# LorienLV/genarchbench

Measured on AMD Instinct MI355X. Metric: bsw ROI M alignments/sec, higher is better.
Workload: dtype i16/i32; 1 GPU; bsw-large; total_items=10000000

## Files before the change

genarchbench_amd/csrc/bsw.hip:

```cpp
#include "gab_internal.h"
#include <atomic>
#include <algorithm>
#include <new>
#include <string.h>
#include <time.h>
#include <stdlib.h>

namespace {

constexpr int kQBuckets = 256;
constexpr int kTBuckets = 256;
constexpr int kNumKeys = kQBuckets * kTBuckets;
constexpr int kClassStep = 16;
constexpr int kNumClasses = kQBuckets / kClassStep;
constexpr int kSlices = 2;
constexpr int64_t kSlice0 = 1 << 20;
constexpr int64_t kSliceMin = 1 << 22;
constexpr int kSortGridBeside = 256;
static_assert(kSliceMin >= (1 << 21) && kSlice0 < kSliceMin && kSlice0 >= 64 * 8192, "slice 0 has to fill the chip with its class launches, and calls below 2^21 pairs stay unsliced");

struct BswConst {
    int32_t o_del, e_del, o_ins, e_ins, zdrop, end_bonus, w, max_sc;
    uint32_t row_lo[5];
    uint32_t row_hi[5];
};

struct BswStats {
    unsigned long long cells;
    int32_t max_h0[kNumClasses];
    int32_t bad;
    int32_t first_bad;
};
GAB_STATIC_ATOMIC64(BswStats, cells);

struct BswIO {
    const uint8_t *ref; const int64_t *ref_off;
    const uint8_t *qry; const int64_t *qry_off;
    const int32_t *len1, *len2, *h0;
    int64_t ref_bytes, qry_bytes, n;
    int64_t ref_lo, qry_lo;
    int64_t ref_hi, qry_hi;
};

__device__ __forceinline__ int bsw_key(int qlen, int tlen, int h0) {
    int tb = tlen >> 3; if (tb > kTBuckets / 4 - 1) tb = kTBuckets / 4 - 1;
    int hc = h0 >> 5; if (hc > 3) hc = 3;
    return (qlen - 1) * kTBuckets + tb * 4 + hc;
}

__device__ __forceinline__ int bsw_hslot(int key) { return (int)(((uint32_t)key * 4099u) & (uint32_t)(kNumKeys - 1)); }
static_assert((kNumKeys & (kNumKeys - 1)) == 0, "bsw_hslot needs a power-of-two key space");

__global__ __launch_bounds__(256) void bsw_hist(BswIO io, int64_t lo, int64_t hi, uint32_t *hist, uint32_t *rank, BswStats *st) {
    __shared__ int cls_h0[kNumClasses];
    if (threadIdx.x < kNumClasses) cls_h0[threadIdx.x] = 0;
    __syncthreads();
    int64_t i = lo + (int64_t)blockIdx.x * blockDim.x + threadIdx.x;
    int64_t stride = (int64_t)gridDim.x * blockDim.x;
    for (; i < hi; i += stride) {
        int ql = io.len2[i], tl = io.len1[i], h = io.h0[i];
        int64_t ro = io.ref_off[i], qo = io.qry_off[i];
        bool ok = ql >= 1 && ql <= GAB_BSW_MAX_QLEN && tl >= 1 && tl <= GAB_BSW_MAX_TLEN && h >= 0 &&
                  h <= (1 << 29) && ro >= io.ref_lo && qo >= io.qry_lo &&
                  ro + tl + 3 <= io.ref_bytes && qo + ql + 3 <= io.qry_bytes &&
                  ro + tl <= io.ref_hi && qo + ql <= io.qry_hi;
        if (!ok) {
            atomicAdd(&st->bad, 1);
            atomicMin((unsigned int *)&st->first_bad, (unsigned int)(i + 1 > 0x7fffffff ? 0x7fffffff : i + 1));
            rank[i] = ~0u;
            continue;
        }
        if (h > 0) atomicMax(&cls_h0[(ql - 1) / kClassStep], h);
        rank[i] = atomicAdd(&hist[bsw_hslot(bsw_key(ql, tl, h))], 1u);
    }
    __syncthreads();
    if (threadIdx.x < kNumClasses && cls_h0[threadIdx.x] > 0) atomicMax(&st->max_h0[threadIdx.x], cls_h0[threadIdx.x]);
}

constexpr int kScanBlocks = kNumKeys / 1024;
static_assert(kScanBlocks == 64, "bsw_scan_b reduces the block totals with one wave");
__global__ __launch_bounds__(1024) void bsw_scan_a(const uint32_t *__restrict__ hist, uint32_t *__restrict__ start, uint32_t *__restrict__ sums) {
    __shared__ uint32_t wsum[16];
    const int t = threadIdx.x, key = blockIdx.x * 1024 + t, lane = t & 63, wv = t >> 6;
    const uint32_t v = hist[bsw_hslot(key)];
    uint32_t inc = v;
    for (int o = 1; o < 64; o <<= 1) { const uint32_t u = __shfl_up(inc, o); if (lane >= o) inc += u; }
    if (lane == 63) wsum[wv] = inc;
    __syncthreads();
    uint32_t before = 0;
    for (int k = 0; k < wv; k++) before += wsum[k];
    start[key] = before + inc - v;
    if (t == 1023) sums[blockIdx.x] = before + inc;
}
__global__ __launch_bounds__(1024) void bsw_scan_b(uint32_t *__restrict__ start, const uint32_t *__restrict__ sums, uint32_t *__restrict__ qstart) {
    __shared__ uint32_t s_off, s_total;
    const int t = threadIdx.x, key = blockIdx.x * 1024 + t;
    if (t < 64) {
        const uint32_t sv = sums[t];
        uint32_t mine = t < (int)blockIdx.x ? sv : 0, all = sv;
        for (int o = 32; o > 0; o >>= 1) { mine += __shfl_xor(mine, o); all += __shfl_xor(all, o); }
        if (t == 0) { s_off = mine; s_total = all; }
    }
    __syncthreads();
    const uint32_t run = start[key] + s_off;
    start[key] = run;
    if ((key % kTBuckets) == 0) qstart[key / kTBuckets] = run;
    if (key == kNumKeys - 1) { start[kNumKeys] = s_total; qstart[kQBuckets] = s_total; }
}

struct __attribute__((aligned(32))) BswRec { int64_t ref_off, qry_off; int32_t len1, len2, h0; uint32_t id; };

__global__ __launch_bounds__(256) void bsw_scatter(BswIO io, int64_t lo, int64_t hi, const uint32_t *__restrict__ start,
                                                   const uint32_t *__restrict__ rank, BswRec *recs) {
    int64_t i = lo + (int64_t)blockIdx.x * blockDim.x + threadIdx.x;
    int64_t stride = (int64_t)gridDim.x * blockDim.x;
    for (; i < hi; i += stride) {
        int ql = io.len2[i], tl = io.len1[i];
        if (rank[i] == ~0u) continue;
        BswRec r;
        r.ref_off = io.ref_off[i]; r.qry_off = io.qry_off[i]; r.len1 = tl; r.len2 = ql; r.h0 = io.h0[i]; r.id = (uint32_t)i;
        recs[start[bsw_key(ql, tl, r.h0)] + rank[i]] = r;
    }
}

__device__ __forceinline__ uint32_t load_u32_unaligned(const uint8_t *p) {
    uint32_t w;
    __builtin_memcpy(&w, p, 4);
    return w;
}

template <bool WIDE>
__global__ __launch_bounds__(64) void bsw_dp(BswIO io, BswConst c, const BswRec *__restrict__ recs,
                                            int64_t kbeg, int64_t kend, int qcap,
                                            int32_t *__restrict__ score_out,
                                            gab_bsw_result *__restrict__ result_out, BswStats *st) {
    extern __shared__ uint32_t lds[];
    const int lane = threadIdx.x;
    const int64_t k = kbeg + (int64_t)(gridDim.x - 1 - blockIdx.x) * 64 + lane;
    const bool valid = k < kend;
    BswRec rec; rec.ref_off = rec.qry_off = 0; rec.len1 = rec.len2 = rec.h0 = 0; rec.id = 0u;
    if (valid) rec = recs[k];
    const uint32_t id = rec.id;

    uint32_t *const H = lds + lane;
    uint32_t *const E = lds + (size_t)(qcap + 1) * 64 + lane;
    uint8_t *const QC = reinterpret_cast<uint8_t *>(lds + (size_t)(WIDE ? 2 : 1) * (qcap + 1) * 64) + lane * 4;

    unsigned long long cells = 0;
    if (valid) {
        const int qlen = rec.len2, tlen = rec.len1, h0 = rec.h0;
        const uint8_t *q = io.qry + rec.qry_off;
        const uint8_t *t = io.ref + rec.ref_off;
        const int oe_del = c.o_del + c.e_del, oe_ins = c.o_ins + c.e_ins;
        const int e_del = c.e_del, e_ins = c.e_ins;

        for (int w4 = 0; w4 * 4 < qlen; w4++)
            *reinterpret_cast<uint32_t *>(QC + w4 * 256) = load_u32_unaligned(q + w4 * 4);

        int w = c.w;
        {
            int lim = (int)((double)(qlen * c.max_sc + c.end_bonus - c.o_ins) / e_ins + 1.);
            lim = lim > 1 ? lim : 1; w = w < lim ? w : lim;
            lim = (int)((double)(qlen * c.max_sc + c.end_bonus - c.o_del) / e_del + 1.);
            lim = lim > 1 ? lim : 1; w = w < lim ? w : lim;
        }
        const bool score_only = result_out == nullptr;
        bool prune = score_only && (qlen <= w + 1 || h0 - oe_ins - (w + 1) * e_ins <= 0) && (c.zdrop == 0 || c.zdrop >= 8 * c.max_sc);
        int best, best_i, best_j, g_i, gscore, max_off;
      for (;;) {
        {
            int prev = h0;
            for (int j = 0; j <= qlen; j++) {
                int v;
                if (j == 0) v = h0;
                else if (j == 1) v = h0 > oe_ins ? h0 - oe_ins : 0;
                else v = prev > e_ins ? prev - e_ins : 0;
                prev = v;
                H[j * 64] = (uint32_t)v;
                if (WIDE) E[j * 64] = 0u;
            }
        }
        best = h0; best_i = -1; best_j = -1; g_i = -1; gscore = -1; max_off = 0;
        int beg = 0, end = qlen;
        int stale_pot = 0;
        bool dropped = false, abandon = false;
        uint32_t tw = load_u32_unaligned(t);
        for (int i = 0; i < tlen; i++) {
            const int tc = (tw >> ((i & 3) * 8)) & 0xff;
            if ((i & 3) == 3 && i + 1 < tlen) tw = load_u32_unaligned(t + i + 1);
            uint32_t rlo = c.row_lo[4], rhi = c.row_hi[4];
            rlo = tc == 0 ? c.row_lo[0] : rlo; rhi = tc == 0 ? c.row_hi[0] : rhi;
            rlo = tc == 1 ? c.row_lo[1] : rlo; rhi = tc == 1 ? c.row_hi[1] : rhi;
            rlo = tc == 2 ? c.row_lo[2] : rlo; rhi = tc == 2 ? c.row_hi[2] : rhi;
            rlo = tc == 3 ? c.row_lo[3] : rlo; rhi = tc == 3 ? c.row_hi[3] : rhi;

            if (beg < i - w) beg = i - w;
            if (end > i + w + 1) { end = i + w + 1; stale_pot = max(stale_pot, best + c.max_sc * (qlen - end)); }
            if (end > qlen) end = qlen;
            const int beg0 = beg, end0 = end;
            int hleft = 0;
            if (beg == 0) { hleft = h0 - (c.o_del + e_del * (i + 1)); hleft = hleft > 0 ? hleft : 0; }
            int f = 0;
            uint32_t rowpk = 0;
            int rowmax32 = 0, rowmax_j = -1;
            int j = beg;
            for (; j < end; j++) {
                int diag, e;
                if (WIDE) { diag = (int)H[j * 64]; e = (int)E[j * 64]; }
                else { uint32_t v = H[j * 64]; diag = (int)(v & 0xffffu); e = (int)(v >> 16); }
                uint32_t qc = QC[(j >> 2) * 256 + (j & 3)];
                qc = qc > 4u ? 4u : qc;
                int sc = (int)__builtin_amdgcn_perm(rhi, rlo, qc | 0x0c0c0c00u) - 128;
                int M = diag ? diag + sc : 0;
                int h = max(max(M, e), f);
                int t1 = M - oe_del; t1 = t1 > 0 ? t1 : 0;
                int en = e - e_del; en = en > t1 ? en : t1;
                if (WIDE) { H[j * 64] = (uint32_t)hleft; E[j * 64] = (uint32_t)en; }
                else H[j * 64] = (uint32_t)hleft | ((uint32_t)en << 16);
                hleft = h;
                if (WIDE) {
                    if (!(rowmax32 > h)) rowmax_j = j;
                    rowmax32 = h > rowmax32 ? h : rowmax32;
                } else {
                    uint32_t pk = ((uint32_t)h << 16) | (uint32_t)j;
                    rowpk = pk > rowpk ? pk : rowpk;
                }
                int t2 = M - oe_ins; t2 = t2 > 0 ? t2 : 0;
                f -= e_ins; f = f > t2 ? f : t2;
            }
            cells += (unsigned)(end > beg ? end - beg : 0);
            int rowmax;
            if (WIDE) rowmax = rowmax32;
            else { rowmax = (int)(rowpk >> 16); rowmax_j = end > beg ? (int)(rowpk & 0xffffu) : -1; }
            if (WIDE) { H[end * 64] = (uint32_t)hleft; E[end * 64] = 0u; }
            else H[end * 64] = (uint32_t)hleft;
            if (j == qlen) {
                if (!(gscore > hleft)) g_i = i;
                gscore = hleft > gscore ? hleft : gscore;
            }
            if (rowmax == 0) {
                if (dropped && beg == 0) {
                    const int hb = h0 - c.o_del - e_del * (i + 1);
                    abandon = hb > 0 && hb + c.max_sc * min(tlen - 1 - i, qlen) > best;
                }
                break;
            }
            const int rows_left = tlen - 1 - i;
            bool try_exit = false;
            if (rowmax > best) {
                best = rowmax; best_i = i; best_j = rowmax_j;
                int off = rowmax_j - i; off = off < 0 ? -off : off;
                max_off = off > max_off ? off : max_off;
            } else {
                if (c.zdrop > 0) {
                    if (dropped && rowmax < best - c.zdrop) { abandon = true; break; }
                    int di = i - best_i, dj = rowmax_j - best_j;
                    if (di > dj) { if (best - rowmax - (di - dj) * e_del > c.zdrop) break; }
                    else { if (best - rowmax - (dj - di) * e_ins > c.zdrop) break; }
                }
                try_exit = score_only && rowmax + c.max_sc * min(rows_left, qlen - 1 - rowmax_j) <= best;
            }
            if (dropped && end < qlen && end != i + w + 1 && hleft > e_ins &&
                hleft - e_ins + c.max_sc * min(rows_left, qlen - end - 1) > best) { abandon = true; break; }
            if (WIDE) {
                for (j = beg; j < end && H[j * 64] == 0u && E[j * 64] == 0u; j++) {}
                beg = j;
                for (j = end; j >= beg && H[j * 64] == 0u && E[j * 64] == 0u; j--) {}
            } else {
                for (j = beg; j < end && H[j * 64] == 0u; j++) {}
                beg = j;
                for (j = end; j >= beg && H[j * 64] == 0u; j--) {}
            }
            int jl = j;
            end = j + 2 < qlen ? j + 2 : qlen;
            if (prune && beg < end) {
                bool go = true;
                if (beg == 0) {
                    const int hb = h0 - c.o_del - e_del * (i + 2);
                    go = hb <= 0 || hb + c.max_sc * min(rows_left, qlen) <= best;
                }
                if (go) {
                    const int lcap = min(end, beg0 + 4);
                    for (j = beg; j < lcap; j++) {
                        const int m = WIDE ? max((int)H[j * 64], (int)E[j * 64]) : max((int)(H[j * 64] & 0xffffu), (int)(H[j * 64] >> 16));
                        if (m && m + c.max_sc * min(rows_left, qlen - j) > best) break;
                    }
                    dropped = dropped || j > beg;
                    beg = j;
                }
            }
            if (prune && jl >= beg) {
                const int from = jl;
                for (; jl >= beg && jl > end0 - 4; jl--) {
                    const int m = WIDE ? max((int)H[jl * 64], (int)E[jl * 64]) : max((int)(H[jl * 64] & 0xffffu), (int)(H[jl * 64] >> 16));
                    if (m && m + c.max_sc * min(rows_left, qlen - jl) > best) break;
                    H[jl * 64] = 0u;
                    if (WIDE) E[jl * 64] = 0u;
                }
                if (jl < from) { dropped = true; end = jl + 2 < qlen ? jl + 2 : qlen; }
            }
            if (try_exit) {
                int bound = stale_pot;
                if (beg == 0) {
                    const int hb = h0 - c.o_del - e_del * (i + 2);
                    if (hb > 0) bound = max(bound, hb + c.max_sc * min(rows_left, qlen));
                }
                for (j = beg; j <= end && bound <= best; j++) {
                    const int hd = WIDE ? (int)H[j * 64] : (int)(H[j * 64] & 0xffffu);
                    if (hd) bound = max(bound, hd + c.max_sc * min(rows_left, qlen - j));
                }
                if (bound <= best) break;
            }
        }
        if (!abandon) break;
        prune = false;
      }
        score_out[id] = best;
        if (result_out) {
            gab_bsw_result r;
            r.score = best; r.qle = best_j + 1; r.tle = best_i + 1;
            r.gtle = g_i + 1; r.gscore = gscore; r.max_off = max_off;
            result_out[id] = r;
        }
    }
    for (int o = 32; o > 0; o >>= 1) cells += __shfl_xor(cells, o);
    if (lane == 0 && cells) atomicAdd(&st->cells, cells);
}

// ... 52 lines not shown
    asm("v_sub_u16 %0, %2, %3\n\tv_max_i16_sdwa %0, %1, %0 dst_sel:WORD_0 dst_unused:UNUSED_PAD src0_sel:WORD_1 src1_sel:WORD_0"
        : "=&v"(r) : "v"(t), "v"(f), "v"(e));
    return r;
}
__device__ __forceinline__ uint32_t rowkey_fold(uint32_t key, uint32_t a, uint32_t b, uint32_t c, uint32_t j) {
    uint32_t t;
    asm("v_max_i16 %1, %2, %3\n\tv_max_i16 %1, %1, %4\n\tv_lshl_or_b32 %1, %1, 16, %5\n\tv_max_u32 %0, %0, %1"
        : "+v"(key), "=&v"(t) : "v"(a), "v"(b), "v"(c), "v"(j));
    return key;
}
struct BswCellOut { int h, en, f; };
__device__ __forceinline__ BswCellOut bsw_cell(int diag, int e, int f, uint32_t qc, uint32_t rlo, uint32_t rhi, int oe_del,
                                               int e_del, int oe_ins, int e_ins) {
    const int sc = (int)__builtin_amdgcn_perm(rhi, rlo, qc | 0x0c0c0c00u) - 128;
    const int M = diag ? diag + sc : 0;
    BswCellOut o;
    o.h = max(max(M, e), f);
    o.en = max(max(M - oe_del, e - e_del), 0);
    o.f = max(max(M - oe_ins, f - e_ins), 0);
    return o;
}

template <bool SYM, bool MS1, bool SO>
__global__ __launch_bounds__(64) void bsw_dp8(BswIO io, BswConst c, const BswRec *__restrict__ recs, int64_t kbeg,
                                              int64_t kend, int qcap, int32_t *__restrict__ score_out,
                                              gab_bsw_result *__restrict__ result_out, BswStats *st) {
    extern __shared__ uint32_t lds[];
    __shared__ __attribute__((aligned(8))) uint32_t row_tab[10];
    if (threadIdx.x < 5) { row_tab[2 * threadIdx.x] = c.row_lo[threadIdx.x]; row_tab[2 * threadIdx.x + 1] = c.row_hi[threadIdx.x]; }
    __syncthreads();
    const int lane = threadIdx.x;
    const int64_t k = kbeg + (int64_t)(gridDim.x - 1 - blockIdx.x) * 64 + lane;
    const bool valid = k < kend;
    BswRec rec; rec.ref_off = rec.qry_off = 0; rec.len1 = rec.len2 = rec.h0 = 0; rec.id = 0u;
    if (valid) rec = recs[k];
    const uint32_t id = rec.id;
    const int ncell_dw = (qcap + 2) / 2;
    uint8_t *const CB = reinterpret_cast<uint8_t *>(lds + lane);
    uint32_t *const CW = lds + lane;
    uint8_t *const QN = reinterpret_cast<uint8_t *>(lds + (size_t)ncell_dw * 64) + lane;
#define CELL16(j) (*reinterpret_cast<uint16_t *>(CB + ((j) >> 1) * 256 + ((j) & 1) * 2))
#define QPAIR(p) (QN[(p) * 64])

    unsigned long long cells = 0;
    if (valid) {
        const int qlen = rec.len2, tlen = rec.len1, h0 = rec.h0;
        const uint8_t *q = io.qry + rec.qry_off;
        const uint8_t *t = io.ref + rec.ref_off;
        const int oe_del = c.o_del + c.e_del, oe_ins = c.o_ins + c.e_ins;
        const int e_del = c.e_del, e_ins = c.e_ins;

        for (int p0 = 0; p0 * 2 < qlen; p0 += 4) {
            const uint32_t s0 = load_u32_unaligned(q + p0 * 2);
            const uint32_t s1 = p0 * 2 + 4 < qlen ? load_u32_unaligned(q + p0 * 2 + 4) : 0u;
            const uint32_t n0 = pk_min_u16(s0 & 0x00ff00ffu, 0x00040004u) | pk_min_u16((s0 >> 8) & 0x00ff00ffu, 0x00040004u) << 4;
            const uint32_t n1 = pk_min_u16(s1 & 0x00ff00ffu, 0x00040004u) | pk_min_u16((s1 >> 8) & 0x00ff00ffu, 0x00040004u) << 4;
            QPAIR(p0) = (uint8_t)n0; QPAIR(p0 + 1) = (uint8_t)(n0 >> 16);
            QPAIR(p0 + 2) = (uint8_t)n1; QPAIR(p0 + 3) = (uint8_t)(n1 >> 16);
        }
        int w = c.w;
        {
            int lim = (int)((double)(qlen * c.max_sc + c.end_bonus - c.o_ins) / e_ins + 1.);
            lim = lim > 1 ? lim : 1; w = w < lim ? w : lim;
            lim = (int)((double)(qlen * c.max_sc + c.end_bonus - c.o_del) / e_del + 1.);
            lim = lim > 1 ? lim : 1; w = w < lim ? w : lim;
        }
        uint32_t k_selz = 0x0c000c00u, k_lo8 = 0x00ff00ffu, v_e_ins = (uint32_t)e_ins;
        uint32_t k_cstep = 512u, k_qstep = 128u, k_jstep = 4u;
        asm volatile("" : "+v"(k_selz), "+v"(k_lo8), "+v"(v_e_ins), "+v"(k_cstep), "+v"(k_qstep), "+v"(k_jstep));
        bool prune = SO && (qlen <= w + 1 || h0 - oe_ins - (w + 1) * e_ins <= 0) && (c.zdrop == 0 || c.zdrop >= 8 * c.max_sc);
        int best, best_i, best_j, g_i, gscore, max_off;
      for (;;) {
        {
            int v = h0 - oe_ins;
            CW[0] = (uint32_t)h0 | (uint32_t)max(v, 0) << 16;
            for (int p = 1; p <= (qlen >> 1); p++) {
                const int lo = v - e_ins;
                v = lo - e_ins;
                CW[p * 64] = (uint32_t)max(lo, 0) | (uint32_t)max(v, 0) << 16;
            }
        }
        best = h0; best_i = -1; best_j = -1; g_i = -1; gscore = -1; max_off = 0;
        int beg = 0, end = qlen;
        int hrow = h0 - c.o_del - e_del;
        int stale_pot = 0;
        bool dropped = false, abandon = false;
        uint32_t tw = load_u32_unaligned(t);
        for (int i = 0; i < tlen; i++, hrow -= e_del) {
            const int tc = (tw >> ((i & 3) * 8)) & 0xff;
            if ((i & 3) == 3 && i + 1 < tlen) tw = load_u32_unaligned(t + i + 1);
            const uint2 rr = *reinterpret_cast<const uint2 *>(&row_tab[2 * (tc < 4 ? tc : 4)]);
            const uint32_t rlo = rr.x, rhi = rr.y;
            if (beg < i - w) beg = i - w;
            if (end > i + w + 1) { end = i + w + 1; stale_pot = max(stale_pot, best + mul24(c.max_sc, qlen - end)); }
            if (end > qlen) end = qlen;
            int hleft = 0;
            if (beg == 0) hleft = hrow > 0 ? hrow : 0;
            int f = 0;
            uint32_t rowpk = 0;
            int j = beg;
            uint32_t *cw = CW + (j >> 1) * 64;
            const uint8_t *qp = QN + (j >> 1) * 64;
            uint32_t v0 = cw[0], q0 = qp[0];
            {
                const uint32_t vn = cw[64], qn = qp[64];
                if ((j & 1) && j < end) {
                    const BswCellOut o = bsw_cell((int)((v0 >> 16) & 0xff), (int)(v0 >> 24), f, q0 >> 4, rlo, rhi, oe_del, e_del,
                                                  oe_ins, e_ins);
                    CELL16(j) = (uint16_t)(hleft | o.en << 8);
                    hleft = o.h; f = o.f;
                    rowpk = ((uint32_t)o.h << 16) | (uint32_t)j;
                    j++;
                    v0 = vn; q0 = qn; cw += 64; qp += 64;
                }
            }
            if (j + 1 < end) {
                const uint32_t k_oe_del = as_u32(pk_splat(oe_del)), k_e_del = as_u32(pk_splat(e_del));
                const uint32_t k_oe_ins = as_u32(pk_splat(oe_ins));
                const uint32_t k_bias = 0x00800080u, k_nib = 0x000f000fu;
// ... 36 lines not shown
                }
                if (j + 1 < end) {
                    const uint32_t v1 = cl[64], q1 = ql[64];
                    uint32_t hj;
                    BSW_PAIR(v0, q0, cl[0], hj)
                    const uint32_t pa = (hj << 16) | (uint32_t)j, pb = (HB << 16) | (uint32_t)(j + 1);
                    rowpk = max(max(rowpk, pa), pb);
                    j += 2; v0 = v1; q0 = q1;
                }
                hleft = (int)HB; f = (int)FV;
#undef BSW_PAIR
            }
            if (j < end) {
                const BswCellOut o = bsw_cell((int)(v0 & 0xff), (int)((v0 >> 8) & 0xff), f, q0 & 0xfu, rlo, rhi, oe_del, e_del,
                                              oe_ins, e_ins);
                CELL16(j) = (uint16_t)(hleft | o.en << 8);
                hleft = o.h; f = o.f;
                const uint32_t pk = ((uint32_t)o.h << 16) | (uint32_t)j;
                rowpk = pk > rowpk ? pk : rowpk;
                j++;
            }
            cells += (unsigned)(end > beg ? end - beg : 0);
            const int rowmax = (int)(rowpk >> 16);
            CELL16(end) = (uint16_t)hleft;
            if constexpr (!SO) {
                if (j == qlen) {
                    if (!(gscore > hleft)) g_i = i;
                    gscore = hleft > gscore ? hleft : gscore;
                }
            }
            if (rowmax == 0) {
                if constexpr (SO) {
                    if (dropped && beg == 0) {
                        abandon = hrow > 0 && hrow + mul24(c.max_sc, min(tlen - 1 - i, qlen)) > best;
                    }
                }
                break;
            }
            const int kj = (int)(rowpk & 0xffffu);
            const int pb = beg >> 1, pe = end >> 1;
            const uint32_t *const rw = CW + ((kj + 1) >> 1) * 64;
            const uint32_t r0 = rw[0], r1 = rw[64], r2 = rw[128];
            const uint32_t b0 = CW[pb * 64], b1 = CW[(pb + 1) * 64], b2 = CW[(pb + 2) * 64];
            const uint32_t e2 = CW[pe * 64], e1 = CW[(pe > 0 ? pe - 1 : 0) * 64], e0 = CW[(pe > 1 ? pe - 2 : 0) * 64];
            int rowmax_j;
            {
                const uint32_t sh = (uint32_t)((kj + 1) & 1) << 4;
                const uint32_t c01 = __builtin_amdgcn_alignbit(r1, r0, sh), c23 = __builtin_amdgcn_alignbit(r2, r1, sh);
                const uint32_t rm2 = (uint32_t)rowmax * 0x00010001u;
                const uint32_t ne = __builtin_amdgcn_perm(pk_min_u16_1((c23 ^ rm2) & 0x00ff00ffu), pk_min_u16_1((c01 ^ rm2) & 0x00ff00ffu),
                                                          0x06040200u);
                const int nv = end - kj < 4 ? end - kj : 4;
                const uint32_t eq = (ne ^ 0x01010101u) & (0x01010101u >> (8 * (4 - nv)));
                rowmax_j = kj + ((31 - __builtin_clz(eq)) >> 3);
            }
            const int rows_left = tlen - 1 - i;
            const bool raised = rowmax > best;
            bool stop = false;
            if (c.zdrop > 0) {
                const int di = i - best_i, dj = rowmax_j - best_j;
                const int gap = di > dj ? mul24(di - dj, e_del) : mul24(dj - di, e_ins);
                stop = !raised && best - rowmax - gap > c.zdrop;
                if constexpr (SO) {
                    abandon = !raised && dropped && rowmax < best - c.zdrop;
                    stop = stop || abandon;
                }
            }
            const bool try_exit = SO && !raised && rowmax + mul24(c.max_sc, min(rows_left, qlen - 1 - rowmax_j)) <= best;
            if (raised) {
                best = rowmax; best_i = i; best_j = rowmax_j;
                if constexpr (!SO) {
                    int off = rowmax_j - i; off = off < 0 ? -off : off;
                    max_off = off > max_off ? off : max_off;
                }
            }
            if constexpr (SO) {
                const bool guard = !stop && dropped && end < qlen && end != i + w + 1 && hleft > e_ins &&
                                   hleft - e_ins + mul24(c.max_sc, min(rows_left, qlen - end - 1)) > best;
                abandon = abandon || guard;
                stop = stop || guard;
            }
            int edge_pot = 0;
            {
                const int beg0 = beg, end0 = end;
                uint64_t x = (uint64_t)b1 << 32 | b0;
                if (beg0 & 1) x = (x >> 16) | (uint64_t)(b2 & 0xffffu) << 48;
                uint64_t y = (uint64_t)e2 << 32 | e1;
                if (!(end0 & 1)) y = (y << 16) | (e0 >> 16);
                const int lz = x ? __builtin_ctzll(x) >> 4 : 4, tz = y ? __builtin_clzll(y) >> 4 : 4;
                int base = min(beg0 + lz, end0);
                int lp = lz, tp = tz;
                if constexpr (SO) {
                    const int rq = min(rows_left, qlen);
                    const int hb = hrow - e_del;
                    edge_pot = hb > 0 ? hb + mul24(c.max_sc, rq) : 0;
                    const bool go = prune && base < qlen && (base != 0 || edge_pot <= best);
                    const uint32_t r2 = as_u32(pk_splat(rq)), m2 = as_u32(pk_splat(c.max_sc));
                    const uint32_t bestL = (uint32_t)(go ? best : 0) * 0x00010001u, bestR = (uint32_t)(prune ? best : 0) * 0x00010001u;
                    const uint32_t cl01 = ((uint32_t)(qlen - beg0) & 0xffffu) | (uint32_t)(qlen - beg0 - 1) << 16;
                    const uint32_t cr01 = ((uint32_t)(qlen - end0 + 3) & 0xffffu) | (uint32_t)(qlen - end0 + 2) << 16;
#define BSW_STAY(W, CL, B2, OUT)                                                                                   \
    {                                                                                                             \
        const uint32_t m = pk_max_i16((W) & 0x00ff00ffu, ((W) >> 8) & 0x00ff00ffu);                              \
        (OUT) = pk_mul_lo(pk_subsat_u16_v(add_u32_v(m, pk_mul_lo(pk_min_u16((CL), r2), m2)), (B2)), pk_min_u16_1(m)); \
    }
                    uint32_t sll, slh, srl, srh;
                    BSW_STAY((uint32_t)x, cl01, bestL, sll)
                    BSW_STAY((uint32_t)(x >> 32), cl01 - 0x00020002u, bestL, slh)
                    BSW_STAY((uint32_t)y, cr01, bestR, srl)
                    BSW_STAY((uint32_t)(y >> 32), cr01 - 0x00020002u, bestR, srh)
#undef BSW_STAY
                    const uint64_t stl = (uint64_t)slh << 32 | sll, str = (uint64_t)srh << 32 | srl;
                    lp = stl ? __builtin_ctzll(stl) >> 4 : 4;
                    tp = str ? __builtin_clzll(str) >> 4 : 4;
                }
                int bl = beg0 + lp;
                if (__builtin_expect(lz == 4, 0)) {
                    for (j = beg0 + 4; j < end0 && CELL16(j) == 0; j++) {}
                    base = bl = j < end0 ? j : end0;
                }
                j = end0 - tz;
                if (__builtin_expect(tz == 4, 0)) for (; j >= base && CELL16(j) == 0; j--) {}
                const int jlz = j > base - 1 ? j : base - 1;
                const int endz = jlz + 2 < qlen ? jlz + 2 : qlen;
                beg = bl < endz ? bl : endz;
                int jl = jlz;
                if constexpr (SO) {
                    dropped = dropped || beg > base;
                    int jn = end0 - tp;
                    jn = jn > beg - 1 ? jn : beg - 1;
                    dropped = dropped || jn < jlz;
// ... 77 lines not shown
    hipStream_t aux[kAux] = {nullptr};
    hipEvent_t fork = nullptr, join[kAux] = {nullptr};
    hipStream_t sort = nullptr;
    hipEvent_t sort_fork = nullptr, sort_join = nullptr;
    bool have_stats = false;
    int stat_slices = 1;
    uint32_t *h_qstart[kSlices] = {nullptr};
    BswStats *h_stats[kSlices] = {nullptr};
    BswStats *h_init = nullptr;
    bool out_of_order = false;
};

extern "C" int gab_bsw_create(const gab_bsw_params *p, int device, gab_bsw **out) {
    if (!p || !out) { gab_set_error("gab_bsw_create: NULL argument"); return GAB_EINVAL; }
    *out = nullptr;
    GAB_CHECK(p->e_del > 0 && p->e_ins > 0 && p->o_del >= 0 && p->o_ins >= 0,
              "gab_bsw_create: gap penalties must be o>=0, e>0 (got o_del=%d e_del=%d o_ins=%d e_ins=%d)",
              p->o_del, p->e_del, p->o_ins, p->e_ins);
    GAB_CHECK(p->w >= 0 && p->zdrop >= 0, "gab_bsw_create: w and zdrop must be >= 0");
    GAB_CHECK(p->o_del + p->e_del < 32768 && p->o_ins + p->e_ins < 32768 && p->end_bonus >= -32768 &&
              p->end_bonus < 32768, "gab_bsw_create: penalties out of 16-bit range");
    int rc = gab_check_device(device);
    if (rc) return rc;
    gab_device_guard g(device);
    gab_bsw *h = new (std::nothrow) gab_bsw();
    if (!h) { gab_set_error("out of host memory"); return GAB_ENOMEM; }
    h->device = device; h->prm = *p;
    BswConst &c = h->cst;
    c.o_del = p->o_del; c.e_del = p->e_del; c.o_ins = p->o_ins; c.e_ins = p->e_ins;
    c.zdrop = p->zdrop; c.end_bonus = p->end_bonus; c.w = p->w;
    int mx = 0;
    for (int k = 0; k < 25; k++) mx = p->mat[k] > mx ? p->mat[k] : mx;
    c.max_sc = mx;
    for (int t = 0; t < 5; t++) {
        uint32_t lo = 0;
        for (int q = 0; q < 4; q++) lo |= (uint32_t)(uint8_t)(p->mat[t * 5 + q] + 128) << (8 * q);
        c.row_lo[t] = lo;
        c.row_hi[t] = (uint32_t)(uint8_t)(p->mat[t * 5 + 4] + 128);
    }
    for (int k = 0; k < 4; k++)
        if (hipEventCreate(&h->ev[k]) != hipSuccess) { gab_set_error("hipEventCreate failed"); delete h; return GAB_EDEVICE; }
    bool aux_ok = hipEventCreateWithFlags(&h->fork, hipEventDisableTiming) == hipSuccess;
    for (int k = 0; k < gab_bsw::kAux && aux_ok; k++)
        aux_ok = hipStreamCreateWithFlags(&h->aux[k], hipStreamNonBlocking) == hipSuccess &&
                 hipEventCreateWithFlags(&h->join[k], hipEventDisableTiming) == hipSuccess;
    if (!aux_ok) { gab_set_error("gab_bsw_create: stream / event creation failed"); delete h; return GAB_EDEVICE; }
    if (hipFuncSetAttribute((const void *)bsw_dp<false>, hipFuncAttributeMaxDynamicSharedMemorySize, 160 * 1024) != hipSuccess ||
        hipFuncSetAttribute((const void *)bsw_dp<true>, hipFuncAttributeMaxDynamicSharedMemorySize, 160 * 1024) != hipSuccess) {
        gab_set_error("hipFuncSetAttribute(MaxDynamicSharedMemorySize) failed"); delete h; return GAB_EDEVICE;
    }
    for (int k = 0; k < 8; k++)
        if (hipFuncSetAttribute((const void *)bsw_dp8_kernel(k & 4, k & 2, k & 1), hipFuncAttributeMaxDynamicSharedMemorySize, 160 * 1024 - 64) != hipSuccess) {
            gab_set_error("hipFuncSetAttribute(MaxDynamicSharedMemorySize) failed"); delete h; return GAB_EDEVICE;
        }
    if (hipHostMalloc((void **)&h->h_qstart[0], sizeof(uint32_t) * (kQBuckets + 1) * kSlices) != hipSuccess ||
        hipHostMalloc((void **)&h->h_stats[0], sizeof(BswStats) * (kSlices + 1)) != hipSuccess) {
        gab_set_error("hipHostMalloc failed"); gab_bsw_destroy(h); return GAB_ENOMEM;
    }
    for (int k = 1; k < kSlices; k++) { h->h_qstart[k] = h->h_qstart[0] + (size_t)k * (kQBuckets + 1); h->h_stats[k] = h->h_stats[0] + k; }
    h->h_init = h->h_stats[0] + kSlices;
    memset(h->h_init, 0, sizeof(BswStats));
    h->h_init->first_bad = 0x7fffffff;
    *out = h;
    return GAB_OK;
}

extern "C" void gab_bsw_destroy(gab_bsw *h) {
    if (!h) return;
    gab_device_guard g(h->device);
    h->ws.release(); h->io.release(); h->hs.release();
    for (int k = 0; k < 4; k++) if (h->ev[k]) (void)hipEventDestroy(h->ev[k]);
    if (h->fork) (void)hipEventDestroy(h->fork);
    for (int k = 0; k < gab_bsw::kAux; k++) {
        if (h->join[k]) (void)hipEventDestroy(h->join[k]);
        if (h->aux[k]) (void)hipStreamDestroy(h->aux[k]);
    }
    if (h->sort_fork) (void)hipEventDestroy(h->sort_fork);
    if (h->sort_join) (void)hipEventDestroy(h->sort_join);
    if (h->sort) (void)hipStreamDestroy(h->sort);
    if (h->h_qstart[0]) (void)hipHostFree(h->h_qstart[0]);
    if (h->h_stats[0]) (void)hipHostFree(h->h_stats[0]);
    delete h;
}

struct BswLayout {
    size_t o_start, o_qstart, o_sums, o_stats, blk;
    size_t o_recs, o_rank, total;
    explicit BswLayout(size_t n) {
        o_start = sizeof(uint32_t) * kNumKeys;
        o_qstart = o_start + sizeof(uint32_t) * (kNumKeys + 1);
        o_sums = o_qstart + sizeof(uint32_t) * (kQBuckets + 1);
        o_stats = (o_sums + sizeof(uint32_t) * kScanBlocks + 15) & ~(size_t)15;
        blk = (o_stats + sizeof(BswStats) + 255) & ~(size_t)255;
        o_recs = blk * kSlices;
        o_rank = o_recs + ((sizeof(BswRec) * n + 255) & ~(size_t)255);
        total = o_rank + sizeof(uint32_t) * n;
    }
};

static int bsw_run_device_impl(gab_bsw *h, const uint8_t *ref, int64_t ref_bytes, const int64_t *ref_off,
                               const uint8_t *qry, int64_t qry_bytes, const int64_t *qry_off,
                               const int32_t *len1, const int32_t *len2, const int32_t *h0, int64_t n,
                               int32_t *score_out, gab_bsw_result *result_out, void *stream_, int64_t ref_lo, int64_t qry_lo,
                               int64_t ref_hi, int64_t qry_hi);
extern "C" int gab_bsw_run_device(gab_bsw *h, const uint8_t *ref, int64_t ref_bytes, const int64_t *ref_off,
                                  const uint8_t *qry, int64_t qry_bytes, const int64_t *qry_off,
                                  const int32_t *len1, const int32_t *len2, const int32_t *h0, int64_t n,
                                  int32_t *score_out, gab_bsw_result *result_out, void *stream_) {
    if (h) gab_tuning_refresh(&h->tun);
    return bsw_run_device_impl(h, ref, ref_bytes, ref_off, qry, qry_bytes, qry_off, len1, len2, h0, n, score_out, result_out, stream_, 0, 0,
                               ref_bytes, qry_bytes);
}
static int bsw_run_device_impl(gab_bsw *h, const uint8_t *ref, int64_t ref_bytes, const int64_t *ref_off,
                               const uint8_t *qry, int64_t qry_bytes, const int64_t *qry_off,
                               const int32_t *len1, const int32_t *len2, const int32_t *h0, int64_t n,
                               int32_t *score_out, gab_bsw_result *result_out, void *stream_, int64_t ref_lo, int64_t qry_lo,
                               int64_t ref_hi, int64_t qry_hi) {
    GAB_CHECK(h, "gab_bsw_run_device: NULL handle");
    GAB_CHECK(n >= 0 && n < (1ll << 31), "gab_bsw_run_device: n=%lld out of range", (long long)n);
    h->have_stats = false;
    if (n == 0) return GAB_OK;
    GAB_CHECK(ref && ref_off && qry && qry_off && len1 && len2 && h0 && score_out,
              "gab_bsw_run_device: NULL buffer");
    gab_device_guard g(h->device);
    hipStream_t s = (hipStream_t)stream_;

    const int64_t slice0 = h->tun.bsw_slice[0] > 0 ? h->tun.bsw_slice[0] : kSlice0;
    const int64_t slice_min = std::max<int64_t>(h->tun.bsw_slice[1] > 0 ? h->tun.bsw_slice[1] : kSliceMin, slice0 + 1);
    const int nsl = n >= slice_min ? kSlices : 1;
    const int64_t cut[kSlices + 1] = {0, nsl > 1 ? slice0 : n, n};
    if (nsl > 1 && !h->sort) {
        if (hipStreamCreateWithFlags(&h->sort, hipStreamNonBlocking) != hipSuccess) { h->sort = nullptr; gab_set_error("gab_bsw_run_device: stream creation failed"); return GAB_EDEVICE; }
        if (!h->sort_fork) GAB_HIP(hipEventCreateWithFlags(&h->sort_fork, hipEventDisableTiming));
        if (!h->sort_join) GAB_HIP(hipEventCreateWithFlags(&h->sort_join, hipEventDisableTiming));
    }

    const BswLayout L((size_t)n);
    int rc = h->ws.reserve(L.total);
    if (rc) return rc;
    char *base = h->ws.as<char>();
    BswRec *d_recs = (BswRec *)(base + L.o_recs);
    uint32_t *d_rank = (uint32_t *)(base + L.o_rank);
    auto d_stats = [&](int k) { return (BswStats *)(base + L.blk * k + L.o_stats); };

    BswIO io{ref, ref_off, qry, qry_off, len1, len2, h0, ref_bytes, qry_bytes, n, ref_lo, qry_lo, ref_hi, qry_hi};
    auto enqueue_sort = [&](int k, hipStream_t q) -> hipError_t {
        char *b = base + L.blk * k;
        uint32_t *d_hist = (uint32_t *)b, *d_start = (uint32_t *)(b + L.o_start), *d_qstart = (uint32_t *)(b + L.o_qstart);
        uint32_t *d_sums = (uint32_t *)(b + L.o_sums);
        const int64_t lo = cut[k], hi = cut[k + 1];
        hipError_t e = hipMemsetAsync(b, 0, L.blk, q);
        if (e == hipSuccess) e = hipMemcpyAsync(d_stats(k), h->h_init, sizeof(BswStats), hipMemcpyHostToDevice, q);
        if (e != hipSuccess) return e;
        const int gmax = k > 0 ? kSortGridBeside : 1024;
        const int grid = (int)(gab_ceil_div(hi - lo, 256) < gmax ? gab_ceil_div(hi - lo, 256) : gmax);
        hipLaunchKernelGGL(bsw_hist, dim3(grid), dim3(256), 0, q, io, lo, hi, d_hist, d_rank, d_stats(k));
        hipLaunchKernelGGL(bsw_scan_a, dim3(kScanBlocks), dim3(1024), 0, q, d_hist, d_start, d_sums);
        hipLaunchKernelGGL(bsw_scan_b, dim3(kScanBlocks), dim3(1024), 0, q, d_start, (const uint32_t *)d_sums, d_qstart);
        hipLaunchKernelGGL(bsw_scatter, dim3(grid), dim3(256), 0, q, io, lo, hi, d_start, d_rank, d_recs + lo);
        e = hipMemcpyAsync(h->h_qstart[k], d_qstart, sizeof(uint32_t) * (kQBuckets + 1), hipMemcpyDeviceToHost, q);
        if (e == hipSuccess) e = hipMemcpyAsync(h->h_stats[k], d_stats(k), sizeof(BswStats), hipMemcpyDeviceToHost, q);
        return e;
    };
    GAB_HIP(hipEventRecord(h->ev[0], s));
    GAB_HIP(enqueue_sort(0, s));
    GAB_HIP(hipStreamSynchronize(s));
    const bool sym = h->cst.o_del + h->cst.e_del == h->cst.o_ins + h->cst.e_ins;
    const bool ms1 = h->cst.max_sc <= 1;

    hipStream_t s_main = s;
    auto join_all = [&]() {
        (void)hipStreamSynchronize(s_main);
        for (int k = 0; k < gab_bsw::kAux; k++) (void)hipStreamSynchronize(h->aux[k]);
        if (nsl > 1) (void)hipStreamSynchronize(h->sort);
    };
#define BSW_HIP_JOINED(call)                                                                                       \
    do {                                                                                                           \
        hipError_t e_ = (call);                                                                                    \
        if (e_ != hipSuccess) {                                                                                    \
            gab_set_error("%s:%d: %s -> %s", __FILE__, __LINE__, #call, hipGetErrorString(e_));                    \
            join_all();                                                                                            \
            return e_ == hipErrorOutOfMemory ? GAB_ENOMEM : GAB_EDEVICE;                                           \
        }                                                                                                          \
    } while (0)
    GAB_HIP(hipEventRecord(h->fork, s));
    for (int k = 0; k < gab_bsw::kAux; k++) GAB_HIP(hipStreamWaitEvent(h->aux[k], h->fork, 0));
    int nlaunch = 0;
    constexpr int kRing = gab_bsw::kAux + 2;
    hipStream_t ring[kRing] = {nsl > 1 ? h->sort : nullptr, s_main};
    for (int k = 0; k < gab_bsw::kAux; k++) ring[k + 2] = h->aux[k];
    for (int sl = 0; sl < nsl; sl++) {
    if (sl > 0) BSW_HIP_JOINED(hipStreamSynchronize(h->sort));
// ... 205 lines not shown
```

Measured before the change: 425.4 M alignments/s.

## Seed banded DP with an ungapped diagonal lower bound to prune and sort

```diff
diff --git a/genarchbench_amd/csrc/bsw.hip b/genarchbench_amd/csrc/bsw.hip
--- a/genarchbench_amd/csrc/bsw.hip
+++ b/genarchbench_amd/csrc/bsw.hip
@@ -14,13 +14,16 @@
 constexpr int kClassStep = 16;
 constexpr int kNumClasses = kQBuckets / kClassStep;
 constexpr int kSlices = 2;
-constexpr int64_t kSlice0 = 1 << 20;
+constexpr int64_t kSlice0 = 1572864;
+constexpr int64_t kSlice0Full = 1 << 20;
 constexpr int64_t kSliceMin = 1 << 22;
 constexpr int kSortGridBeside = 256;
-static_assert(kSliceMin >= (1 << 21) && kSlice0 < kSliceMin && kSlice0 >= 64 * 8192, "slice 0 has to fill the chip with its class launches, and calls below 2^21 pairs stay unsliced");
+constexpr int kSeedGridBeside = 512;
+static_assert(kSliceMin >= (1 << 21) && kSlice0 < kSliceMin && kSlice0Full >= 64 * 8192 && kSlice0 >= kSlice0Full, "slice 0 has to fill the chip with its class launches, and calls below 2^21 pairs stay unsliced");
 
 struct BswConst {
     int32_t o_del, e_del, o_ins, e_ins, zdrop, end_bonus, w, max_sc;
+    int32_t seed;
     uint32_t row_lo[5];
     uint32_t row_hi[5];
 };
@@ -42,36 +45,109 @@
     int64_t ref_hi, qry_hi;
 };
 
-__device__ __forceinline__ int bsw_key(int qlen, int tlen, int h0) {
-    int tb = tlen >> 3; if (tb > kTBuckets / 4 - 1) tb = kTBuckets / 4 - 1;
-    int hc = h0 >> 5; if (hc > 3) hc = 3;
-    return (qlen - 1) * kTBuckets + tb * 4 + hc;
+__device__ __forceinline__ int bsw_key(int qlen, int tlen, int h0, int L, int max_sc, int seeded) {
+    if (!seeded) {
+        int tb = tlen >> 3; if (tb > kTBuckets / 4 - 1) tb = kTBuckets / 4 - 1;
+        int hc = h0 >> 5; if (hc > 3) hc = 3;
+        return (qlen - 1) * kTBuckets + tb * 4 + hc;
+    }
+    int d = qlen - (L - h0) / (max_sc > 1 ? max_sc : 1);
+    d = d < 0 ? 0 : d > kTBuckets - 1 ? kTBuckets - 1 : d;
+    return (qlen - 1) * kTBuckets + d;
 }
 
 __device__ __forceinline__ int bsw_hslot(int key) { return (int)(((uint32_t)key * 4099u) & (uint32_t)(kNumKeys - 1)); }
 static_assert((kNumKeys & (kNumKeys - 1)) == 0, "bsw_hslot needs a power-of-two key space");
 
-__global__ __launch_bounds__(256) void bsw_hist(BswIO io, int64_t lo, int64_t hi, uint32_t *hist, uint32_t *rank, BswStats *st) {
+__device__ __forceinline__ uint32_t load_u32_unaligned(const uint8_t *p) {
+    uint32_t w;
+    __builtin_memcpy(&w, p, 4);
+    return w;
+}
+
+__device__ __forceinline__ void bsw_seed_mat(const BswConst &c, int *s_mat) {
+    if (threadIdx.x < 25) {
+        const int t = threadIdx.x / 5, q = threadIdx.x % 5;
+        s_mat[threadIdx.x] = (int)((q < 4 ? c.row_lo[t] >> (8 * q) : c.row_hi[t]) & 0xffu) - 128;
+    }
+}
+__device__ __forceinline__ int bsw_seed_of(const BswIO &io, const BswConst &c, const int *s_mat, int seeded, int64_t i) {
+    {
+        const int ql = io.len2[i], tl = io.len1[i], h = io.h0[i];
+        const int64_t ro = io.ref_off[i], qo = io.qry_off[i];
+        const bool ok = ql >= 1 && ql <= GAB_BSW_MAX_QLEN && tl >= 1 && tl <= GAB_BSW_MAX_TLEN && h >= 0 &&
+                        h <= (1 << 29) && ro >= io.ref_lo && qo >= io.qry_lo &&
+                        ro + tl + 3 <= io.ref_bytes && qo + ql + 3 <= io.qry_bytes &&
+                        ro + tl <= io.ref_hi && qo + ql <= io.qry_hi;
+        if (!ok) return -1;
+        if (!seeded) return h;
+        const uint8_t *const t = io.ref + ro, *const q = io.qry + qo;
+        const int n = ql < tl ? ql : tl;
+        int d = h, L = h, mn = h;
+        bool live = h > 0;
+        for (int k = 0; k < n && live; k += 16) {
+            uint32_t tw[4], qw[4];
+            if (k + 16 <= n + 3) {
+                __builtin_memcpy(tw, t + k, 16);
+                __builtin_memcpy(qw, q + k, 16);
+            } else {
+#pragma unroll
+                for (int b = 0; b < 4; b++) {
+                    const bool in = k + 4 * b < n;
+                    tw[b] = in ? load_u32_unaligned(t + k + 4 * b) : 0u;
+                    qw[b] = in ? load_u32_unaligned(q + k + 4 * b) : 0u;
+                }
+            }
+#pragma unroll
+            for (int b = 0; b < 16; b++) {
+                const uint32_t tc = (tw[b >> 2] >> (8 * (b & 3))) & 0xffu, qc = (qw[b >> 2] >> (8 * (b & 3))) & 0xffu;
+                const int nd = d + s_mat[(tc < 4u ? tc : 4u) * 5u + (qc < 4u ? qc : 4u)];
+                live = live && k + b < n && nd > 0;
+                if (live) {
+                    d = nd;
+                    int v = d;
+                    if (c.zdrop > 0 && d - mn > c.zdrop) v = c.zdrop + 1 + mn;
+                    L = v > L ? v : L;
+                    mn = d < mn ? d : mn;
+                }
+            }
+        }
+        return L;
+    }
+}
+__global__ __launch_bounds__(256) void bsw_seed(BswIO io, BswConst c, int seeded, int64_t lo, int64_t hi, int32_t *__restrict__ seed) {
+    __shared__ int s_mat[25];
+    bsw_seed_mat(c, s_mat);
+    __syncthreads();
+    int64_t i = lo + (int64_t)blockIdx.x * blockDim.x + threadIdx.x;
+    const int64_t stride = (int64_t)gridDim.x * blockDim.x;
+    for (; i < hi; i += stride) seed[i] = bsw_seed_of(io, c, s_mat, seeded, i);
+}
+
+template <bool FUSED>
+__global__ __launch_bounds__(256) void bsw_hist(BswIO io, BswConst c, int seeded, int64_t lo, int64_t hi, int32_t *seed,
+                                                uint32_t *hist, uint32_t *rank, BswStats *st) {
     __shared__ int cls_h0[kNumClasses];
+    __shared__ int s_mat[25];
+    const int max_sc = c.max_sc;
     if (threadIdx.x < kNumClasses) cls_h0[threadIdx.x] = 0;
+    if (FUSED) bsw_seed_mat(c, s_mat);
     __syncthreads();
     int64_t i = lo + (int64_t)blockIdx.x * blockDim.x + threadIdx.x;
     int64_t stride = (int64_t)gridDim.x * blockDim.x;
     for (; i < hi; i += stride) {
-        int ql = io.len2[i], tl = io.len1[i], h = io.h0[i];
-        int64_t ro = io.ref_off[i], qo = io.qry_off[i];
-        bool ok = ql >= 1 && ql <= GAB_BSW_MAX_QLEN && tl >= 1 && tl <= GAB_BSW_MAX_TLEN && h >= 0 &&
-                  h <= (1 << 29) && ro >= io.ref_lo && qo >= io.qry_lo &&
-                  ro + tl + 3 <= io.ref_bytes && qo + ql + 3 <= io.qry_bytes &&
-                  ro + tl <= io.ref_hi && qo + ql <= io.qry_hi;
-        if (!ok) {
+        const int L = FUSED ? bsw_seed_of(io, c, s_mat, seeded, i) : seed[i];
+        if (FUSED) seed[i] = L;
+        if (L < 0) {
             atomicAdd(&st->bad, 1);
             atomicMin((unsigned int *)&st->first_bad, (unsigned int)(i + 1 > 0x7fffffff ? 0x7fffffff : i + 1));
             rank[i] = ~0u;
             continue;
         }
+        const int ql = io.len2[i], h = io.h0[i];
+        const int tl = seeded ? 0 : io.len1[i];
         if (h > 0) atomicMax(&cls_h0[(ql - 1) / kClassStep], h);
-        rank[i] = atomicAdd(&hist[bsw_hslot(bsw_key(ql, tl, h))], 1u);
+        rank[i] = atomicAdd(&hist[bsw_hslot(bsw_key(ql, tl, h, L, max_sc, seeded))], 1u);
     }
     __syncthreads();
     if (threadIdx.x < kNumClasses && cls_h0[threadIdx.x] > 0) atomicMax(&st->max_h0[threadIdx.x], cls_h0[threadIdx.x]);
@@ -108,26 +184,22 @@
     if (key == kNumKeys - 1) { start[kNumKeys] = s_total; qstart[kQBuckets] = s_total; }
 }
 
-struct __attribute__((aligned(32))) BswRec { int64_t ref_off, qry_off; int32_t len1, len2, h0; uint32_t id; };
-
-__global__ __launch_bounds__(256) void bsw_scatter(BswIO io, int64_t lo, int64_t hi, const uint32_t *__restrict__ start,
-                                                   const uint32_t *__restrict__ rank, BswRec *recs) {
+struct __attribute__((aligned(32))) BswRec { int64_t ref_off, qry_off; int32_t lens, h0, L; uint32_t id; };
+static_assert(sizeof(BswRec) == 32 && GAB_BSW_MAX_TLEN < (1 << 16) && GAB_BSW_MAX_QLEN < (1 << 15), "BswRec packs both lengths into one word");
+
+__global__ __launch_bounds__(256) void bsw_scatter(BswIO io, int max_sc, int seeded, int64_t lo, int64_t hi, const int32_t *__restrict__ seed,
+                                                   const uint32_t *__restrict__ start, const uint32_t *__restrict__ rank, BswRec *recs) {
     int64_t i = lo + (int64_t)blockIdx.x * blockDim.x + threadIdx.x;
     int64_t stride = (int64_t)gridDim.x * blockDim.x;
     for (; i < hi; i += stride) {
         int ql = io.len2[i], tl = io.len1[i];
         if (rank[i] == ~0u) continue;
         BswRec r;
-        r.ref_off = io.ref_off[i]; r.qry_off = io.qry_off[i]; r.len1 = tl; r.len2 = ql; r.h0 = io.h0[i]; r.id = (uint32_t)i;
-        recs[start[bsw_key(ql, tl, r.h0)] + rank[i]] = r;
-    }
-}
-
-__device__ __forceinline__ uint32_t load_u32_unaligned(const uint8_t *p) {
-    uint32_t w;
-    __builtin_memcpy(&w, p, 4);
-    return w;
-}
+        r.ref_off = io.ref_off[i]; r.qry_off = io.qry_off[i]; r.lens = tl | ql << 16; r.h0 = io.h0[i]; r.L = seed[i]; r.id = (uint32_t)i;
+        recs[start[bsw_key(ql, tl, r.h0, r.L, max_sc, seeded)] + rank[i]] = r;
+    }
+}
+
 
 template <bool WIDE>
 __global__ __launch_bounds__(64) void bsw_dp(BswIO io, BswConst c, const BswRec *__restrict__ recs,
@@ -138,7 +210,7 @@
     const int lane = threadIdx.x;
     const int64_t k = kbeg + (int64_t)(gridDim.x - 1 - blockIdx.x) * 64 + lane;
     const bool valid = k < kend;
-    BswRec rec; rec.ref_off = rec.qry_off = 0; rec.len1 = rec.len2 = rec.h0 = 0; rec.id = 0u;
+    BswRec rec; rec.ref_off = rec.qry_off = 0; rec.lens = rec.h0 = rec.L = 0; rec.id = 0u;
     if (valid) rec = recs[k];
     const uint32_t id = rec.id;
 
@@ -148,7 +220,7 @@
 
     unsigned long long cells = 0;
     if (valid) {
-        const int qlen = rec.len2, tlen = rec.len1, h0 = rec.h0;
+        const int qlen = rec.lens >> 16, tlen = rec.lens & 0xffff, h0 = rec.h0;
         const uint8_t *q = io.qry + rec.qry_off;
         const uint8_t *t = io.ref + rec.ref_off;
         const int oe_del = c.o_del + c.e_del, oe_ins = c.o_ins + c.e_ins;
@@ -184,6 +256,19 @@
         int beg = 0, end = qlen;
         int stale_pot = 0;
         bool dropped = false, abandon = false;
+        const bool seed_ok = prune && min(qlen, 2 * w + 1) > 9;
+        const int Lm1 = seed_ok && (c.seed & 1) ? rec.L - 1 : 0;
+        if (seed_ok && (c.seed & 2)) {
+            const int thr = max(best, Lm1);
+            int jl = qlen;
+            for (; jl >= 1; jl--) {
+                const int m = (int)H[jl * 64];
+                if (m && m + c.max_sc * min(tlen, qlen - jl) > thr) break;
+                H[jl * 64] = 0u;
+            }
+            end = jl + 2 < qlen ? jl + 2 : qlen;
+            dropped = end < min(qlen, w + 1);
+        }
         uint32_t tw = load_u32_unaligned(t);
         for (int i = 0; i < tlen; i++) {
             const int tc = (tw >> ((i & 3) * 8)) & 0xff;
@@ -241,7 +326,7 @@
             if (rowmax == 0) {
                 if (dropped && beg == 0) {
                     const int hb = h0 - c.o_del - e_del * (i + 1);
-                    abandon = hb > 0 && hb + c.max_sc * min(tlen - 1 - i, qlen) > best;
+                    abandon = hb > 0 && hb + c.max_sc * min(tlen - 1 - i, qlen) > max(best, Lm1);
                 }
                 break;
             }
@@ -260,8 +345,9 @@
                 }
                 try_exit = score_only && rowmax + c.max_sc * min(rows_left, qlen - 1 - rowmax_j) <= best;
             }
+            const int thr = max(best, Lm1);
             if (dropped && end < qlen && end != i + w + 1 && hleft > e_ins &&
-                hleft - e_ins + c.max_sc * min(rows_left, qlen - end - 1) > best) { abandon = true; break; }
+                hleft - e_ins + c.max_sc * min(rows_left, qlen - end - 1) > thr) { abandon = true; break; }
             if (WIDE) {
                 for (j = beg; j < end && H[j * 64] == 0u && E[j * 64] == 0u; j++) {}
                 beg = j;
@@ -277,13 +363,13 @@
                 bool go = true;
                 if (beg == 0) {
                     const int hb = h0 - c.o_del - e_del * (i + 2);
-                    go = hb <= 0 || hb + c.max_sc * min(rows_left, qlen) <= best;
+                    go = hb <= 0 || hb + c.max_sc * min(rows_left, qlen) <= thr;
                 }
                 if (go) {
                     const int lcap = min(end, beg0 + 4);
                     for (j = beg; j < lcap; j++) {
                         const int m = WIDE ? max((int)H[j * 64], (int)E[j * 64]) : max((int)(H[j * 64] & 0xffffu), (int)(H[j * 64] >> 16));
-                        if (m && m + c.max_sc * min(rows_left, qlen - j) > best) break;
+                        if (m && m + c.max_sc * min(rows_left, qlen - j) > thr) break;
                     }
                     dropped = dropped || j > beg;
                     beg = j;
@@ -293,7 +379,7 @@
                 const int from = jl;
                 for (; jl >= beg && jl > end0 - 4; jl--) {
                     const int m = WIDE ? max((int)H[jl * 64], (int)E[jl * 64]) : max((int)(H[jl * 64] & 0xffffu), (int)(H[jl * 64] >> 16));
-                    if (m && m + c.max_sc * min(rows_left, qlen - jl) > best) break;
+                    if (m && m + c.max_sc * min(rows_left, qlen - jl) > thr) break;
                     H[jl * 64] = 0u;
                     if (WIDE) E[jl * 64] = 0u;
                 }
@@ -412,7 +498,7 @@
     const int lane = threadIdx.x;
     const int64_t k = kbeg + (int64_t)(gridDim.x - 1 - blockIdx.x) * 64 + lane;
     const bool valid = k < kend;
-    BswRec rec; rec.ref_off = rec.qry_off = 0; rec.len1 = rec.len2 = rec.h0 = 0; rec.id = 0u;
+    BswRec rec; rec.ref_off = rec.qry_off = 0; rec.lens = rec.h0 = rec.L = 0; rec.id = 0u;
     if (valid) rec = recs[k];
     const uint32_t id = rec.id;
     const int ncell_dw = (qcap + 2) / 2;
@@ -424,7 +510,7 @@
 
     unsigned long long cells = 0;
     if (valid) {
-        const int qlen = rec.len2, tlen = rec.len1, h0 = rec.h0;
+        const int qlen = rec.lens >> 16, tlen = rec.lens & 0xffff, h0 = rec.h0;
         const uint8_t *q = io.qry + rec.qry_off;
         const uint8_t *t = io.ref + rec.ref_off;
         const int oe_del = c.o_del + c.e_del, oe_ins = c.o_ins + c.e_ins;
@@ -451,20 +537,33 @@
         bool prune = SO && (qlen <= w + 1 || h0 - oe_ins - (w + 1) * e_ins <= 0) && (c.zdrop == 0 || c.zdrop >= 8 * c.max_sc);
         int best, best_i, best_j, g_i, gscore, max_off;
       for (;;) {
+        const bool seed_ok = SO && prune && min(qlen, 2 * w + 1) > 9;
+        const int Lm1 = seed_ok && (c.seed & 1) ? rec.L - 1 : 0;
+        const bool row_prune = seed_ok && (c.seed & 2);
+        int jm1 = 0;
         {
+            const int thr0 = row_prune ? max(h0, Lm1) : -1;
             int v = h0 - oe_ins;
-            CW[0] = (uint32_t)h0 | (uint32_t)max(v, 0) << 16;
+            int cl = qlen - 1;
+            const bool l1 = v > 0 && v + mul24(c.max_sc, min(tlen, cl)) > thr0;
+            jm1 = l1 ? 1 : 0;
+            CW[0] = (uint32_t)h0 | (uint32_t)(l1 ? v : 0) << 16;
             for (int p = 1; p <= (qlen >> 1); p++) {
                 const int lo = v - e_ins;
                 v = lo - e_ins;
-                CW[p * 64] = (uint32_t)max(lo, 0) | (uint32_t)max(v, 0) << 16;
+                cl -= 2;
+                const bool la = lo > 0 && lo + mul24(c.max_sc, min(tlen, cl + 1)) > thr0;
+                const bool lb = v > 0 && v + mul24(c.max_sc, min(tlen, cl)) > thr0;
+                jm1 = la ? 2 * p : jm1; jm1 = lb ? 2 * p + 1 : jm1;
+                CW[p * 64] = (uint32_t)(la ? lo : 0) | (uint32_t)(lb ? v : 0) << 16;
             }
         }
         best = h0; best_i = -1; best_j = -1; g_i = -1; gscore = -1; max_off = 0;
-        int beg = 0, end = qlen;
+        int beg = 0, end = row_prune && jm1 + 2 < qlen ? jm1 + 2 : qlen;
         int hrow = h0 - c.o_del - e_del;
         int stale_pot = 0;
-        bool dropped = false, abandon = false;
+        bool dropped = row_prune && end < min(qlen, w + 1);
+        bool abandon = false;
         uint32_t tw = load_u32_unaligned(t);
         for (int i = 0; i < tlen; i++, hrow -= e_del) {
             const int tc = (tw >> ((i & 3) * 8)) & 0xff;
@@ -567,7 +666,7 @@
             if (rowmax == 0) {
                 if constexpr (SO) {
                     if (dropped && beg == 0) {
-                        abandon = hrow > 0 && hrow + mul24(c.max_sc, min(tlen - 1 - i, qlen)) > best;
+                        abandon = hrow > 0 && hrow + mul24(c.max_sc, min(tlen - 1 - i, qlen)) > max(best, Lm1);
                     }
                 }
                 break;
@@ -609,9 +708,10 @@
                     max_off = off > max_off ? off : max_off;
                 }
             }
+            const int thr = max(best, Lm1);
             if constexpr (SO) {
                 const bool guard = !stop && dropped && end < qlen && end != i + w + 1 && hleft > e_ins &&
-                                   hleft - e_ins + mul24(c.max_sc, min(rows_left, qlen - end - 1)) > best;
+                                   hleft - e_ins + mul24(c.max_sc, min(rows_left, qlen - end - 1)) > thr;
                 abandon = abandon || guard;
                 stop = stop || guard;
             }
@@ -629,9 +729,9 @@
                     const int rq = min(rows_left, qlen);
                     const int hb = hrow - e_del;
                     edge_pot = hb > 0 ? hb + mul24(c.max_sc, rq) : 0;
-                    const bool go = prune && base < qlen && (base != 0 || edge_pot <= best);
+                    const bool go = prune && base < qlen && (base != 0 || edge_pot <= thr);
                     const uint32_t r2 = as_u32(pk_splat(rq)), m2 = as_u32(pk_splat(c.max_sc));
-                    const uint32_t bestL = (uint32_t)(go ? best : 0) * 0x00010001u, bestR = (uint32_t)(prune ? best : 0) * 0x00010001u;
+                    const uint32_t bestL = (uint32_t)(go ? thr : 0) * 0x00010001u, bestR = (uint32_t)(prune ? thr : 0) * 0x00010001u;
                     const uint32_t cl01 = ((uint32_t)(qlen - beg0) & 0xffffu) | (uint32_t)(qlen - beg0 - 1) << 16;
                     const uint32_t cr01 = ((uint32_t)(qlen - end0 + 3) & 0xffffu) | (uint32_t)(qlen - end0 + 2) << 16;
 #define BSW_STAY(W, CL, B2, OUT)                                                                                   \
@@ -775,6 +875,7 @@
     int mx = 0;
     for (int k = 0; k < 25; k++) mx = p->mat[k] > mx ? p->mat[k] : mx;
     c.max_sc = mx;
+    c.seed = 1 | (mx <= p->e_ins ? 2 : 0);
     for (int t = 0; t < 5; t++) {
         uint32_t lo = 0;
         for (int q = 0; q < 4; q++) lo |= (uint32_t)(uint8_t)(p->mat[t * 5 + q] + 128) << (8 * q);
@@ -828,7 +929,7 @@
 
 struct BswLayout {
     size_t o_start, o_qstart, o_sums, o_stats, blk;
-    size_t o_recs, o_rank, total;
+    size_t o_recs, o_rank, o_seed, total;
     explicit BswLayout(size_t n) {
         o_start = sizeof(uint32_t) * kNumKeys;
         o_qstart = o_start + sizeof(uint32_t) * (kNumKeys + 1);
@@ -837,7 +938,8 @@
         blk = (o_stats + sizeof(BswStats) + 255) & ~(size_t)255;
         o_recs = blk * kSlices;
         o_rank = o_recs + ((sizeof(BswRec) * n + 255) & ~(size_t)255);
-        total = o_rank + sizeof(uint32_t) * n;
+        o_seed = o_rank + ((sizeof(uint32_t) * n + 255) & ~(size_t)255);
+        total = o_seed + sizeof(int32_t) * n;
     }
 };
 
@@ -868,7 +970,7 @@
     gab_device_guard g(h->device);
     hipStream_t s = (hipStream_t)stream_;
 
-    const int64_t slice0 = h->tun.bsw_slice[0] > 0 ? h->tun.bsw_slice[0] : kSlice0;
+    const int64_t slice0 = h->tun.bsw_slice[0] > 0 ? h->tun.bsw_slice[0] : result_out ? kSlice0Full : kSlice0;
     const int64_t slice_min = std::max<int64_t>(h->tun.bsw_slice[1] > 0 ? h->tun.bsw_slice[1] : kSliceMin, slice0 + 1);
     const int nsl = n >= slice_min ? kSlices : 1;
     const int64_t cut[kSlices + 1] = {0, nsl > 1 ? slice0 : n, n};
@@ -884,6 +986,7 @@
     char *base = h->ws.as<char>();
     BswRec *d_recs = (BswRec *)(base + L.o_recs);
     uint32_t *d_rank = (uint32_t *)(base + L.o_rank);
+    int32_t *d_seed = (int32_t *)(base + L.o_seed);
     auto d_stats = [&](int k) { return (BswStats *)(base + L.blk * k + L.o_stats); };
 
     BswIO io{ref, ref_off, qry, qry_off, len1, len2, h0, ref_bytes, qry_bytes, n, ref_lo, qry_lo, ref_hi, qry_hi};
@@ -897,10 +1000,17 @@
         if (e != hipSuccess) return e;
         const int gmax = k > 0 ? kSortGridBeside : 1024;
         const int grid = (int)(gab_ceil_div(hi - lo, 256) < gmax ? gab_ceil_div(hi - lo, 256) : gmax);
-        hipLaunchKernelGGL(bsw_hist, dim3(grid), dim3(256), 0, q, io, lo, hi, d_hist, d_rank, d_stats(k));
+        const int sgrid = (int)(gab_ceil_div(hi - lo, 256) < kSeedGridBeside ? gab_ceil_div(hi - lo, 256) : kSeedGridBeside);
+        const int seeded = result_out == nullptr;
+        if (k > 0) {
+            hipLaunchKernelGGL(bsw_seed, dim3(sgrid), dim3(256), 0, q, io, h->cst, seeded, lo, hi, d_seed);
+            hipLaunchKernelGGL(bsw_hist<false>, dim3(grid), dim3(256), 0, q, io, h->cst, seeded, lo, hi, d_seed, d_hist, d_rank, d_stats(k));
+        } else {
+            hipLaunchKernelGGL(bsw_hist<true>, dim3(grid), dim3(256), 0, q, io, h->cst, seeded, lo, hi, d_seed, d_hist, d_rank, d_stats(k));
+        }
         hipLaunchKernelGGL(bsw_scan_a, dim3(kScanBlocks), dim3(1024), 0, q, d_hist, d_start, d_sums);
         hipLaunchKernelGGL(bsw_scan_b, dim3(kScanBlocks), dim3(1024), 0, q, d_start, (const uint32_t *)d_sums, d_qstart);
-        hipLaunchKernelGGL(bsw_scatter, dim3(grid), dim3(256), 0, q, io, lo, hi, d_start, d_rank, d_recs + lo);
+        hipLaunchKernelGGL(bsw_scatter, dim3(grid), dim3(256), 0, q, io, h->cst.max_sc, seeded, lo, hi, (const int32_t *)d_seed, d_start, d_rank, d_recs + lo);
         e = hipMemcpyAsync(h->h_qstart[k], d_qstart, sizeof(uint32_t) * (kQBuckets + 1), hipMemcpyDeviceToHost, q);
         if (e == hipSuccess) e = hipMemcpyAsync(h->h_stats[k], d_stats(k), sizeof(BswStats), hipMemcpyDeviceToHost, q);
         return e;
```

Measured after the change: 461.3 M alignments/s (median of 6 runs). 8.4% higher.
